# qiyu3816/DiffSG

Hardware: AMD Instinct MI355X
Metric: ddpm_reverse_sample_steps_per_sec_msr80c (higher is better)
Workload: dtype f32(2xf16-split MFMA, f32 accumulate); 1 GPU; MSR-80c CFG reverse sampling, batch 65536 x D=C=80 per GPU, UNet1D(proj 128, dims (64,32,16,8), n_blocks 2), omega=1, device Philox noise; rows sharded, no collective; batch_per_gpu=65536, solution_dim=80, parallelism=rows x1

## Files before the change

### diffsg_amd/csrc/dsg_panel.hpp

```cpp
#pragma once
#include "dsg_wide.hpp"

namespace dsg {

constexpr int kPW = 8;
constexpr int kPanelU4 = 2048;
constexpr int kPrivU4 = 128;
constexpr int kPrivSlots = 5;
constexpr int kPrivDist = 4;
constexpr int kPanelLdsU4 = 2 * kPanelU4 + kPW * kPrivSlots * kPrivU4 + kWideVec / 4;
constexpr int panel_pw(int steps) { return 2 * steps; }
constexpr int panel_u4(int steps) { return 512 * steps; }
constexpr int panel_lds_u4(int steps) { return 2 * panel_u4(steps) + panel_pw(steps) * kPrivSlots * kPrivU4 + kWideVec / 4; }

#ifndef DSG_STAMP_DBG
#define DSG_STAMP_DBG 0
#endif
#ifndef DSG_STAMP_DOWN0
#define DSG_STAMP_DOWN0 0
#endif
#ifdef DSG_CYCLE_STAMPS
constexpr int kPanelStampU4 = kPW * 128 / 2;
#define DSG_PSTAMP(tag)                                                                                               \
    do {                                                                                                              \
        if (STAMPED && blockIdx.x == 0 && stamp_k < 128) {                                                           \
            const unsigned long long t_ = __builtin_readcyclecounter();                                               \
            if (lane == 0 && !(DSG_STAMP_DBG & 1)) stamp_lds[wave * 128 + stamp_k] = (t_ << 16) | (unsigned long long)(tag); \
            if (DSG_STAMP_DBG & 1) asm volatile("" :: "s"(t_));                                                       \
            ++stamp_k;                                                                                                \
        }                                                                                                             \
    } while (0)
#else
constexpr int kPanelStampU4 = 0;
#define DSG_PSTAMP(tag) do {} while (0)
#endif

__device__ __forceinline__ void glds_quad_s(unsigned voff, const void* sbase, unsigned lds_dst) {
    unsigned keep;
    asm volatile("s_mov_b32 %0, m0\n\ts_mov_b32 m0, %3\n\ts_nop 0\n\t"
                 "global_load_lds_dwordx4 %1, %2\n\t"
                 "global_load_lds_dwordx4 %1, %2 offset:1024\n\t"
                 "global_load_lds_dwordx4 %1, %2 offset:2048\n\t"
                 "global_load_lds_dwordx4 %1, %2 offset:3072\n\t"
                 "s_mov_b32 m0, %0"
                 : "=&s"(keep) : "v"(voff), "s"(sbase), "s"(lds_dst) : "memory");
}
__device__ __forceinline__ void glds_pair_s(unsigned voff, const void* sbase, unsigned lds_dst) {
    unsigned keep;
    asm volatile("s_mov_b32 %0, m0\n\ts_mov_b32 m0, %3\n\ts_nop 0\n\t"
                 "global_load_lds_dwordx4 %1, %2\n\t"
                 "global_load_lds_dwordx4 %1, %2 offset:1024\n\t"
                 "s_mov_b32 m0, %0"
                 : "=&s"(keep) : "v"(voff), "s"(sbase), "s"(lds_dst) : "memory");
}
__device__ __forceinline__ void glds_stats_s(unsigned voff4, const void* s0, const void* s1, unsigned lds_dst) {
    unsigned keep;
    const void* s1m = reinterpret_cast<const char*>(s1) - 256;
    asm volatile("s_mov_b32 %0, m0\n\ts_mov_b32 m0, %4\n\ts_nop 0\n\t"
                 "global_load_lds_dword %1, %2\n\t"
                 "global_load_lds_dword %1, %3 offset:256\n\t"
                 "s_mov_b32 m0, %0"
                 : "=&s"(keep) : "v"(voff4), "s"(s0), "s"(s1m), "s"(lds_dst) : "memory");
}

struct TilePtrs {
    const char *x0, *x1, *cp;
    const char *st0, *st1;
    bool cond;
};
template <bool SCLIN, int PW = kPW>
__device__ __forceinline__ TilePtrs tile_ptrs(const BlockArgs& a, int g, int wave) {
    const int traw = g * PW + wave;
    const int tile = traw < a.ntiles ? traw : a.ntiles - 1;
    const int ptile = tile >= a.tiles_per_pass ? tile - a.tiles_per_pass : tile;
    const int t0 = seg_tile(a.in0, tile), t1 = seg_tile(a.in1, tile);
    TilePtrs t;
    t.x0 = reinterpret_cast<const char*>(a.in0.data + (size_t)t0 * 16 * 256);
    t.st0 = reinterpret_cast<const char*>(a.in0.stats + (size_t)t0 * 64);
    t.x1 = SCLIN ? reinterpret_cast<const char*>(a.in1.data + (size_t)t1 * 16 * 256) : t.x0;
    t.st1 = SCLIN ? reinterpret_cast<const char*>(a.in1.stats + (size_t)t1 * 64) : t.st0;
    t.cp = reinterpret_cast<const char*>(a.cond_pre + (size_t)ptile * 16 * 256);
    t.cond = tile >= a.uncond_tiles;
    return t;
}

struct PanelCtx {
    unsigned lane16, lane4;
    unsigned w_lds;
    unsigned w_rd;
    unsigned p_lds;
    const uint4* wrd;
    const uint4* prd;
    int q;
    int islot, cslot;
};

__device__ __forceinline__ void priv_issue(PanelCtx& c, const char* src) {
    glds_pair_s(c.lane16, src, c.p_lds + (unsigned)c.islot * 2048u);
    c.islot = c.islot == kPrivSlots - 1 ? 0 : c.islot + 1;
}
__device__ __forceinline__ void priv_issue_stats(PanelCtx& c, const char* st0, const char* st1) {
    glds_stats_s(c.lane4, st0, st1, c.p_lds + (unsigned)c.islot * 2048u);
    c.islot = c.islot == kPrivSlots - 1 ? 0 : c.islot + 1;
}
__device__ __forceinline__ const uint4* priv_consume(PanelCtx& c) {
    asm volatile("s_waitcnt vmcnt(6)" ::: "memory");
    const uint4* rd = c.prd + c.cslot * kPrivU4;
    c.cslot = c.cslot == kPrivSlots - 1 ? 0 : c.cslot + 1;
    return rd;
}

template <int NT>
__device__ __forceinline__ void panel_wfrag(HFrag<NT>& w, const uint4* panel , int steps_per_tile, int s) {
#pragma unroll
    for (int nt = 0; nt < NT; ++nt) { w.hi[nt] = panel[(nt * steps_per_tile + s) * 128]; w.lo[nt] = panel[(nt * steps_per_tile + s) * 128 + 64]; }
// ... 150 lines not shown
    if (HASN) {
        constexpr int L0 = 4 * NJ;
        asm volatile("" : "+v"(hq[L0 + 3]), "+v"(lq[L0 + 3]));
        const f32x4 hv = {hq[L0], hq[L0 + 1], hq[L0 + 2], hq[L0 + 3]}, lv = {lq[L0], lq[L0 + 1], lq[L0 + 2], lq[L0 + 3]};
        bcarry.hi = __builtin_bit_cast(h8, hv); bcarry.lo = __builtin_bit_cast(h8, lv);
    }
}

#ifndef DSG_PANEL_TRAIL_PRIO
#define DSG_PANEL_TRAIL_PRIO 1
#endif

template <int STEPS, bool STAMPED>
struct PanelWg {
    static constexpr int N = 128, NT = 4, NG = 16;
    static constexpr int PW = panel_pw(STEPS), PU4 = panel_u4(STEPS), NTHR = 64 * PW;
    static constexpr float kL2 = -1.44269504088896341f;
    int lane, h, j, wave;
    float *g1v, *b1v, *g2v, *b2v, *g3v, *b3v, *tbv, *c2v, *c3v, *gLv, *bLv, *biasLv;
    PanelCtx c;
    int since_w;
#ifdef DSG_CYCLE_STAMPS
    unsigned long long* stamp_lds;
    int stamp_k;
    unsigned long long clk_t0, clk_r0;
#endif
    __device__ __forceinline__ void stamp(int tag) { DSG_PSTAMP(tag); }

    __device__ __forceinline__ void init(uint4* lds) {
        lane = threadIdx.x & 63; h = lane >> 5; j = lane & 31;
        wave = __builtin_amdgcn_readfirstlane(threadIdx.x >> 6);
#ifdef DSG_CYCLE_STAMPS
        stamp_lds = reinterpret_cast<unsigned long long*>(lds + panel_lds_u4(STEPS));
        stamp_k = 0;
        clk_t0 = __builtin_readcyclecounter(); clk_r0 = __builtin_amdgcn_s_memrealtime();
#endif
        if (STEPS == 4 && wave >= 4) __builtin_amdgcn_s_setprio(DSG_PANEL_TRAIL_PRIO);
        float* const vec = reinterpret_cast<float*>(lds + 2 * PU4 + PW * kPrivSlots * kPrivU4);
        float* const v2 = vec + 2 * kLnLdsW1;
        g1v = vec; b1v = vec + kLnLdsW1;
        g2v = v2; b2v = v2 + 128; g3v = v2 + 256; b3v = v2 + 384; tbv = v2 + 512; c2v = v2 + 640; c3v = v2 + 768;
        gLv = v2 + 896; bLv = v2 + 1024; biasLv = v2 + 1152;
        const unsigned lds0 = (unsigned)(unsigned long long)(const __attribute__((address_space(3))) void*)lds;
        c.lane16 = (unsigned)lane * 16u; c.lane4 = (unsigned)lane * 4u;
        c.w_lds = lds0 + (unsigned)wave * 4096u;
        c.w_rd = lds0 + (unsigned)lane * 16u;
        c.p_lds = lds0 + 2u * PU4 * 16u + (unsigned)wave * (kPrivSlots * 2048u);
        c.wrd = lds + lane;
        c.prd = lds + 2 * PU4 + wave * (kPrivSlots * kPrivU4) + lane;
        c.q = 0; c.islot = 0; c.cslot = 0;
        since_w = 0;
    }

    template <typename More>
    __device__ __forceinline__ void stage_vectors(const BlockArgs& a, More&& more) {
        const int n1 = ln1_extent(a);
        for (int i = threadIdx.x; i < n1; i += NTHR) { g1v[i] = a.gamma1[i] * kL2; b1v[i] = a.beta1[i] * kL2; }
        if (threadIdx.x < 128) {
            const int i = threadIdx.x;
            g2v[i] = a.gamma2[i] * kL2; b2v[i] = a.beta2[i] * kL2; g3v[i] = a.gamma3[i] * kL2; b3v[i] = a.beta3[i] * kL2;
            c2v[i] = a.c2[i]; c3v[i] = a.c3[i];
            tbv[i] = a.tbias[(size_t)(a.step_ptr ? *a.step_ptr : 0) * a.tb_stride + i];
            more(i);
        }
        __syncthreads();
    }

    __device__ __forceinline__ void prologue(const char* st0, const char* st1, const char* x0, const uint4* panel0) {
        priv_issue_stats(c, st0, st1);
        priv_issue(c, x0);
        priv_issue(c, x0 + 2048);
        priv_issue(c, x0 + 4096);
        glds_quad_s(c.lane16, panel0, c.w_lds);
    }

    __device__ __forceinline__ int panel_begin(const uint4* next) {
        if (since_w >= 8) asm volatile("s_waitcnt vmcnt(8) lgkmcnt(0)" ::: "memory");
        else if (STEPS < 4 && since_w >= 4) asm volatile("s_waitcnt vmcnt(4) lgkmcnt(0)" ::: "memory");
        else if (since_w >= 2) asm volatile("s_waitcnt vmcnt(2) lgkmcnt(0)" ::: "memory");
        else asm volatile("s_waitcnt vmcnt(0) lgkmcnt(0)" ::: "memory");
        __builtin_amdgcn_s_barrier();
        const int rd = c.q & 1;
        glds_quad_s(c.lane16, next, c.w_lds + (unsigned)((c.q + 1) & 1) * (PU4 * 16u));
        since_w = 0;
        ++c.q;
        return rd;
    }

    __device__ __forceinline__ BOp step0_mem(const uint4* rd, const float* gv, const float* bv, float cc, float dd) {
        const float4 xa = __builtin_bit_cast(float4, rd[0]), xb = __builtin_bit_cast(float4, rd[64]);
        const float x[8] = {xa.x, xa.y, xa.z, xa.w, xb.x, xb.y, xb.z, xb.w};
        return panel_prep<true, true>(x, gv, bv, 0, cc, dd, h);
    }
    __device__ __forceinline__ BOp step0_reg(const f32x16 (&in)[NT], const float* gv, const float* bv, float cc, float dd) {
        const float x[8] = {in[0][0], in[0][1], in[0][2], in[0][3], in[0][4], in[0][5], in[0][6], in[0][7]};
        return panel_prep<true, true>(x, gv, bv, 0, cc, dd, h);
    }
    static __device__ __forceinline__ const uint4* no_consume(int) { return nullptr; }
    static __device__ __forceinline__ const uint4* none_n() { return nullptr; }

    template <int P1, typename Consume, typename Refill>
    __device__ __forceinline__ void stage1(f32x16 (&acc1)[NT], BOp b0, float cc, float dd, Consume&& consume_s1, Refill&& refill) {
#pragma unroll
        for (int p = 0; p < P1; ++p) {
            const int bi = panel_begin(refill(p));
            stamp(0x14);
            BOp bc;
            const NextPrep nx{&acc1, STEPS * (p + 1), g1v, b1v, cc, dd, nullptr, nullptr};
            auto cs = [&](int jj) { return consume_s1(STEPS * p + 1 + jj); };
            auto cn = [&]() { return consume_s1(STEPS * p + STEPS); };
            if (p + 1 < P1) {
                if (p == 0) panel_pipe_s<true, PIPE_LN, PIPE_LN, STEPS>(acc1, c.wrd + bi * PU4, b0, bc, acc1, STEPS * p, g1v, b1v, cc, dd, h, cs, nx, cn);
                else panel_pipe_s<false, PIPE_LN, PIPE_LN, STEPS>(acc1, c.wrd + bi * PU4, b0, bc, acc1, STEPS * p, g1v, b1v, cc, dd, h, cs, nx, cn);
                b0 = bc;
            } else {
                if (p == 0) panel_pipe_s<true, PIPE_LN, PIPE_NONE, STEPS>(acc1, c.wrd + bi * PU4, b0, bc, acc1, STEPS * p, g1v, b1v, cc, dd, h, cs, nx, none_n);
                else panel_pipe_s<false, PIPE_LN, PIPE_NONE, STEPS>(acc1, c.wrd + bi * PU4, b0, bc, acc1, STEPS * p, g1v, b1v, cc, dd, h, cs, nx, none_n);
            }
// ... 42 lines not shown
    template <typename Ahead>
    __device__ __forceinline__ void priv_add8(f32x16 (&acc)[NT], Ahead&& ahead) {
#pragma unroll
        for (int i = 0; i < 8; ++i) {
            const uint4* rd = priv_consume(c);
            const float4 v0 = __builtin_bit_cast(float4, rd[0]), v1 = __builtin_bit_cast(float4, rd[64]);
            ahead(i);
            acc_add_f4<NT>(acc, 2 * i, v0);
            acc_add_f4<NT>(acc, 2 * i + 1, v1);
        }
    }

    __device__ __forceinline__ void stats_store(const f32x16 (&acc)[NT], const BlockArgs& a, int tile, bool store, float& xmean, float& xm2) {
        acc_stats<N, NT>(acc, h, xmean, xm2);
        if (store) {
            if (h == 0) reinterpret_cast<float2*>(a.out_stats)[(size_t)tile * 32 + j] = make_float2(xmean, xm2);
            acc_store<NG, NT>(acc, a.out + (size_t)tile * NG * 256 + lane * 4);
        }
    }

    __device__ __forceinline__ void finish() {
        asm volatile("s_waitcnt vmcnt(0)" ::: "memory");
#ifdef DSG_CYCLE_STAMPS
        if (STAMPED && blockIdx.x == 0) {
            asm volatile("s_waitcnt lgkmcnt(0)" ::: "memory");
            for (int k = lane; k < 128; k += 64) dsg_stamp_buf[wave * 128 + k] = k < stamp_k ? stamp_lds[wave * 128 + k] : 0ull;
            if (threadIdx.x == 0) {
                dsg_stamp_buf[kPW * 128 + 0] = clk_t0; dsg_stamp_buf[kPW * 128 + 1] = clk_r0;
                dsg_stamp_buf[kPW * 128 + 2] = __builtin_readcyclecounter(); dsg_stamp_buf[kPW * 128 + 3] = __builtin_amdgcn_s_memrealtime();
                dsg_stamp_n = kPW * 128 + 4;
            }
        }
#endif
    }
};

template <bool SCLIN, int EPI, int NTO, int STEPS = 4>
__global__ __launch_bounds__(64 * panel_pw(STEPS), 2) void k_panel128_h(const BlockLinArgsH A, const int ngroups) {
    constexpr int NT = 4;
    constexpr int PW = panel_pw(STEPS), PU4 = panel_u4(STEPS);
    constexpr int KS1 = SCLIN ? 16 : 8, P1 = KS1 / STEPS, P2 = 8 / STEPS, NE = SCLIN ? 16 : 8;
    constexpr int NTOP = NTO <= 1 ? 1 : (NTO == 2 ? 2 : 4), ESTEPS = 4 * STEPS / NTOP;
    constexpr int EPANELS = EPI == 0 ? 0 : (ESTEPS >= 8 ? 1 : 8 / ESTEPS);
    constexpr int PA = P1, PB = PA + P2, PD = PB + P2, PE = PD + (SCLIN ? P1 : 0), NP = PE + EPANELS;
    __shared__ uint4 lds[panel_lds_u4(STEPS) + (STEPS == 4 ? kPanelStampU4 : 0)];
    PanelWg<STEPS, ((DSG_STAMP_DOWN0 ? !SCLIN : SCLIN) && EPI == 0 && STEPS == 4)> w;
    w.init(lds);
    PanelCtx& c = w.c;
    int& since_w = w.since_w;
    const BlockArgsH& ah = A.b;
    const BlockArgs& a = ah.b;
    const int lane = w.lane, h = w.h, j = w.j, wave = w.wave;
    const int stride = gridDim.x;
    w.stage_vectors(a, [&](int i) {
        if (EPI == 2) { w.gLv[i] = A.l.l.gamma[i] * w.kL2; w.bLv[i] = A.l.l.beta[i] * w.kL2; }
        if (EPI != 0) w.biasLv[i] = i < NTO * 32 ? A.l.l.bias[i] : 0.f;
    });
    const float inv1 = ah.kc[0], inv2 = ah.kc[1], inv3 = ah.kc[2];
    float invL = 0.f;
    if (EPI != 0) invL = A.l.kc[EPI == 2 ? 1 : 0];

    const int wnt = wave / (STEPS / 2), wsub = wave % (STEPS / 2);
    const uint4* const w1p = ah.W1h + ((size_t)wnt * KS1) * 128 + wsub * 256;
    const uint4* const w2p = ah.W2h + ((size_t)wnt * 8) * 128 + wsub * 256;
    const uint4* const w3p = ah.W3h + ((size_t)wnt * 8) * 128 + wsub * 256;
    const uint4* const wsp = SCLIN ? ah.Wsch + ((size_t)wnt * KS1) * 128 + wsub * 256 : w1p;
    const uint4* wlp = w1p;
    if (EPI != 0) {
        if (NTOP == 4) wlp = A.l.Wh + ((size_t)(wnt < NTO ? wnt : 0) * 8) * 128 + wsub * 256;
        else if (NTOP == 2) wlp = A.l.Wh + ((size_t)(wave / STEPS) * 8) * 128 + (wave % STEPS) * 256;
        else wlp = A.l.Wh + (wave & 3) * 256;
    }
    auto panel_src = [&](int p) -> const uint4* {
        if (p < PA) return w1p + (size_t)p * (128 * STEPS);
        if (p < PB) return w2p + (size_t)(p - PA) * (128 * STEPS);
        if (p < PD) return w3p + (size_t)(p - PB) * (128 * STEPS);
        if (p < PE) return wsp + (size_t)(p - PD) * (128 * STEPS);
        return wlp + (ESTEPS < 8 ? (size_t)(p - PE) * (128 * ESTEPS) : 0);
    };
    {
        const TilePtrs cur = tile_ptrs<SCLIN, PW>(a, blockIdx.x < ngroups ? blockIdx.x : 0, wave);
        w.prologue(cur.st0, cur.st1, cur.x0, panel_src(0));
    }
    auto xin = [&](const TilePtrs& t, int S) -> const char* { return SCLIN && S >= 8 ? t.x1 + (size_t)(S - 8) * 2048 : t.x0 + (size_t)S * 2048; };

    constexpr bool XT = SCLIN && EPI == 0;
    BOp bcar;
    float cc_car = 0.f, dd_car = 0.f;
    for (int g = blockIdx.x; g < ngroups; g += stride) {
        const int tile_raw = g * PW + wave;
        const bool live = tile_raw < a.ntiles;
        const int tile = live ? tile_raw : a.ntiles - 1;
        const int ptile = tile >= a.tiles_per_pass ? tile - a.tiles_per_pass : tile;
        const TilePtrs cur = tile_ptrs<SCLIN, PW>(a, g, wave);
        const bool my_cond = cur.cond;
        const TilePtrs nxt = tile_ptrs<SCLIN, PW>(a, g + stride < ngroups ? g + stride : g, wave);
        w.stamp(0x01);
        auto issue_tail = [&](int T) {
            if (T < NE) priv_issue(c, xin(cur, T));
            else if (T == NE) priv_issue_stats(c, nxt.st0, nxt.st1);
            else priv_issue(c, nxt.x0 + (size_t)(T - NE - 1) * 2048);
            since_w += 2;
        };
        auto consume_s1 = [&](int S) -> const uint4* {
            const uint4* rd = priv_consume(c);
            if (S + 4 < KS1) { priv_issue(c, xin(cur, S + 4)); since_w += 2; }
            else if (my_cond) { priv_issue(c, cur.cp + (size_t)(S + 4 - KS1) * 2048); since_w += 2; }
            else issue_tail(S + 4 - KS1);
            return rd;
        };
        auto consume_sc = [&](int S) -> const uint4* {
            const uint4* rd = priv_consume(c);
            issue_tail(S + 4);
            return rd;
        };

        auto ln1_stats = [&](const TilePtrs& t, float& cc, float& dd) {
            const uint4* rd = priv_consume(c);
            const float2* sp = reinterpret_cast<const float2*>(rd - lane);
            const float2 s0 = sp[j];
            float mean = s0.x, m2 = s0.y;
            if (SCLIN) {
                const float2 s1 = sp[32 + j];
                const float dd_ = s1.x - mean;
                m2 = m2 + s1.y + dd_ * dd_ * a.chan_w;
                mean = mean + dd_ * a.chan_f;
            }
            priv_issue(c, t.x0 + 3 * 2048); since_w += 2;
            const float rstd = rsqrtf(m2 * a.inv_nin + kLnEps);
            if (SCLIN) range_check(a.range_flag, mean, m2);
            cc = rstd; dd = -mean * rstd;
        };

        f32x16 acc1[NT];
        {
            float cc, dd;
// ... 106 lines not shown
                if (S == 0) mfma_step_h0<NTO>(acc, wf, bhi, blo); else mfma_step_h<NTO>(acc, wf, bhi, blo);
            }
        }
        acc_unscale_add_lds<NTO>(acc, invL, w.biasLv, h);
        if (!live) continue;
        if (EPI == 1) {
            const int NGo = (la.out_width + 7) / 8;
            float m, sq;
            lin_out_stats<NTO>(acc, h, la.out_width, la.inv_out_w, m, sq);
            if (h == 0) reinterpret_cast<float2*>(la.out_stats)[(size_t)tile * 32 + j] = make_float2(m, sq);
#pragma unroll
            for (int G = 0; G < NTO * 4; ++G)
                if (G < NGo) st4(la.out + ((size_t)tile * NGo + G) * 256 + lane * 4, acc_f4<NTO>(acc, G));
        } else {
            const int pass = tile >= la.tiles_per_pass ? 1 : 0, row = ptile * 32 + j;
            if (row < la.nrows) {
                float* o = la.out_rm + ((size_t)pass * la.nrows + row) * la.out_width;
                if ((la.out_width & 3) == 0) {
#pragma unroll
                    for (int G = 0; G < NTO * 4; ++G) {
                        const int f = 8 * G + 4 * h;
                        if (f < la.out_width) st4(o + f, acc_f4<NTO>(acc, G));
                    }
                } else {
#pragma unroll
                    for (int G = 0; G < NTO * 4; ++G)
#pragma unroll
                        for (int qq = 0; qq < 4; ++qq) {
                            const int f = 8 * G + 4 * h + qq;
                            if (f < la.out_width) o[f] = acc[G >> 2][4 * (G & 3) + qq];
                        }
                }
            }
        }
    }
    w.finish();
}

template <int STEPS = 4>
__global__ __launch_bounds__(64 * panel_pw(STEPS), 2) void k_panel128_duo_h(const BlockArgsH ah, const int ngroups) {
    constexpr int NT = 4;
    constexpr int PW = panel_pw(STEPS);
    constexpr int P = 8 / STEPS;
    constexpr int PA = P, PB = 2 * P, PD = 3 * P, NP = 4 * P;
    __shared__ uint4 lds[panel_lds_u4(STEPS) + (STEPS == 4 ? kPanelStampU4 : 0)];
    PanelWg<STEPS, (DSG_STAMP_DOWN0 && STEPS == 4)> w;
    w.init(lds);
    PanelCtx& c = w.c;
    int& since_w = w.since_w;
    const BlockArgs& a = ah.b;
    const int lane = w.lane, h = w.h, j = w.j, wave = w.wave;
    const int stride = gridDim.x;
    const int tpp = a.tiles_per_pass;
    w.stage_vectors(a, [](int) {});
    const float inv1 = ah.kc[0], inv2 = ah.kc[1], inv3 = ah.kc[2];

    const int wnt = wave / (STEPS / 2), wsub = wave % (STEPS / 2);
    const uint4* const w1p = ah.W1h + ((size_t)wnt * 8) * 128 + wsub * 256;
    const uint4* const w2p = ah.W2h + ((size_t)wnt * 8) * 128 + wsub * 256;
    const uint4* const w3p = ah.W3h + ((size_t)wnt * 8) * 128 + wsub * 256;
    auto panel_src = [&](int p) -> const uint4* {
        if (p < PA) return w1p + (size_t)p * (128 * STEPS);
        if (p < PB) return w2p + (size_t)(p - PA) * (128 * STEPS);
        if (p < PD) return w3p + (size_t)(p - PB) * (128 * STEPS);
        return w3p + (size_t)(p - PD) * (128 * STEPS);
    };
    struct RowPtrs { const char *x0, *st0, *cp; };
    auto row_ptrs = [&](int g) -> RowPtrs {
        const int raw = g * PW + wave, pt = raw < tpp ? raw : tpp - 1;
        return RowPtrs{reinterpret_cast<const char*>(a.in0.data + (size_t)pt * 16 * 256), reinterpret_cast<const char*>(a.in0.stats + (size_t)pt * 64),
                       reinterpret_cast<const char*>(a.cond_pre + (size_t)pt * 16 * 256)};
    };
    {
        const RowPtrs cur = row_ptrs(blockIdx.x < ngroups ? blockIdx.x : 0);
        w.prologue(cur.st0, cur.st0, cur.x0, panel_src(0));
    }

    for (int g = blockIdx.x; g < ngroups; g += stride) {
        const int row_raw = g * PW + wave;
        const bool live = row_raw < tpp;
        const int ptile = live ? row_raw : tpp - 1;
        const RowPtrs cur = row_ptrs(g);
        const RowPtrs nxt = row_ptrs(g + stride < ngroups ? g + stride : g);
        w.stamp(0x01);
        auto issue_at = [&](int T) {
            if (T < 8) priv_issue(c, cur.x0 + (size_t)T * 2048);
            else if (T < 16) priv_issue(c, cur.cp + (size_t)(T - 8) * 2048);
            else if (T < 24) priv_issue(c, cur.x0 + (size_t)(T - 16) * 2048);
            else if (T == 24) priv_issue_stats(c, nxt.st0, nxt.st0);
            else priv_issue(c, nxt.x0 + (size_t)(T - 25) * 2048);
            since_w += 2;
        };
        auto consume_s1 = [&](int S) -> const uint4* {
            const uint4* rd = priv_consume(c);
            if (S + 4 < 8) { priv_issue(c, cur.x0 + (size_t)(S + 4) * 2048); since_w += 2; }
            else issue_at(S + 4 - 8);
            return rd;
        };

        f32x16 acc1[NT];
        {
            float cc, dd;
            {
                const uint4* rd = priv_consume(c);
                const float2 s0 = reinterpret_cast<const float2*>(rd - lane)[j];
                priv_issue(c, cur.x0 + 3 * 2048); since_w += 2;
                const float rstd = rsqrtf(s0.y * a.inv_nin + kLnEps);
                cc = rstd; dd = -s0.x * rstd;
            }
            w.stamp(0x10);
            BOp b0 = w.step0_mem(consume_s1(0), w.g1v, w.b1v, cc, dd);
            asm volatile("" : "+v"(b0.hi), "+v"(b0.lo));
            w.stamp(0x11);
            w.template stage1<P>(acc1, b0, cc, dd, consume_s1, [&](int p) { return panel_src(p + 1); });
        }
        acc_unscale_add_lds<NT>(acc1, inv1, w.tbv, h);
        w.stamp(0x13);

        f32x16 acc2[NT];
        {
            float cc, dd;
            BOp b0 = w.template reg_head<0x20>(acc1, w.g2v, w.b2v, cc, dd);
            w.template reg_panels<P - 1, 0x20>(acc2, acc1, w.g2v, w.b2v, cc, dd, b0, [&](int p) { return panel_src(PA + p + 1); });
            w.template reg_last<0x20>(acc2, acc1, w.g2v, w.b2v, cc, dd, b0, panel_src(PA + P));
            acc_unscale_add_lds<NT>(acc2, inv2, w.c2v, h);
        }
        w.stamp(0x23);

        f32x16 (&acc3)[NT] = acc1;
// ... 91 lines not shown
```

### diffsg_amd/csrc/dsg_res64.hpp

```cpp
#pragma once
#include "dsg_panel.hpp"

namespace dsg {

constexpr int kR64Waves = 8;
typedef unsigned u32x4 __attribute__((ext_vector_type(4)));
typedef __attribute__((address_space(3))) const u32x4 lds_cu4;

template <bool SCLIN, int NTO = 0> struct R64Layout {
    static constexpr int KS1 = SCLIN ? 8 : 4;
    static constexpr int W1 = 0, W2 = W1 + 2 * KS1 * 128, W3 = W2 + 2 * 4 * 128, WSC = W3 + 2 * 4 * 128, WL = WSC + (SCLIN ? 2 * KS1 * 128 : 0),
                         VEC = WL + NTO * 4 * 128;
    static constexpr int G1 = 0, B1 = 16 * KS1, G2 = 2 * 16 * KS1, B2 = G2 + 64, G3 = B2 + 64, B3 = G3 + 64, TB = B3 + 64, C2 = TB + 64, C3 = C2 + 64,
                         BL = C3 + 64, NV = BL + 32 * NTO;
    static constexpr int TOTAL_U4 = VEC + (NV + 3) / 4;
};

template <bool LNACT>
__device__ __forceinline__ void r64_prep(const float (&x)[8], const float* gv, const float* bv, int S, float c, float d, int h, h8& hi, h8& lo) {
    const BOp o = panel_prep<LNACT>(x, gv, bv, S, c, d, h);
    hi = o.hi; lo = o.lo;
}

struct R64Planes { u32x4 h0, l0, h1, l1; };
__device__ __forceinline__ R64Planes r64_planes(lds_cu4* w, int tile_stride) { return R64Planes{w[0], w[64], w[tile_stride], w[tile_stride + 64]}; }
struct R64Vec { f32x4 g0, b0, g1, b1; };
__device__ __forceinline__ R64Vec r64_vec(const float* gv, const float* bv, int S, int h) {
    lds_cf4* const gl = (lds_cf4*)(gv + 4 * h);
    lds_cf4* const bl = (lds_cf4*)(bv + 4 * h);
    return R64Vec{gl[4 * S], bl[4 * S], gl[4 * S + 2], bl[4 * S + 2]};
}
template <bool FIRST>
__device__ __forceinline__ void r64_mma_p(f32x16 (&acc)[2], const R64Planes& p, const h8 bhi, const h8 blo) {
    if (FIRST) {
        const f32x16 z = {0.f, 0.f, 0.f, 0.f, 0.f, 0.f, 0.f, 0.f, 0.f, 0.f, 0.f, 0.f, 0.f, 0.f, 0.f, 0.f};
        acc[0] = __builtin_amdgcn_mfma_f32_32x32x16_f16(__builtin_bit_cast(h8, p.h0), bhi, z, 0, 0, 0);
        acc[1] = __builtin_amdgcn_mfma_f32_32x32x16_f16(__builtin_bit_cast(h8, p.h1), bhi, z, 0, 0, 0);
    } else {
        DSG_MFMA_H(acc[0], __builtin_bit_cast(h8, p.h0), bhi);
        DSG_MFMA_H(acc[1], __builtin_bit_cast(h8, p.h1), bhi);
    }
    DSG_MFMA_H(acc[0], __builtin_bit_cast(h8, p.h0), blo);
    DSG_MFMA_H(acc[1], __builtin_bit_cast(h8, p.h1), blo);
    DSG_MFMA_H(acc[0], __builtin_bit_cast(h8, p.l0), bhi);
    DSG_MFMA_H(acc[1], __builtin_bit_cast(h8, p.l1), bhi);
}
template <bool LNACT>
__device__ __forceinline__ void r64_prep_v(const float (&x)[8], const R64Vec& vv, float c, float d, h8& hi, h8& lo) {
    float v[8];
    if (LNACT) {
        constexpr float kk = -1.44269504088896341f / kActScale;
        const float g[8] = {vv.g0[0], vv.g0[1], vv.g0[2], vv.g0[3], vv.g1[0], vv.g1[1], vv.g1[2], vv.g1[3]};
        const float b[8] = {vv.b0[0], vv.b0[1], vv.b0[2], vv.b0[3], vv.b1[0], vv.b1[1], vv.b1[2], vv.b1[3]};
#pragma unroll
        for (int q = 0; q < 8; ++q) {
            const float u = fmaf(fmaf(x[q], c, d), g[q], b[q]);
            v[q] = u * __builtin_amdgcn_rcpf(fmaf(__builtin_amdgcn_exp2f(u), kk, kk));
        }
// ... 38 lines not shown
                __builtin_amdgcn_sched_group_barrier(0x008, 1, 0);
                __builtin_amdgcn_sched_group_barrier(0x002, LNACT ? 11 : 4, 0);
            }
        }
        __builtin_amdgcn_sched_barrier(0);
        pc = pn; bh = nh; bl = nl;
    }
}

template <int NQ>
__device__ __forceinline__ void r64_unscale_add(f32x16 (&acc)[2], float inv, const float* vec, int h) {
    lds_cf4* const v = (lds_cf4*)(vec + 4 * h);
#pragma unroll
    for (int nt = 0; nt < 2; ++nt)
#pragma unroll
        for (int q = 0; q < 4; ++q) {
            const f32x4 b = v[8 * nt + 2 * q];
            acc[nt][4 * q + 0] = fmaf(acc[nt][4 * q + 0], inv, b[0]); acc[nt][4 * q + 1] = fmaf(acc[nt][4 * q + 1], inv, b[1]);
            acc[nt][4 * q + 2] = fmaf(acc[nt][4 * q + 2], inv, b[2]); acc[nt][4 * q + 3] = fmaf(acc[nt][4 * q + 3], inv, b[3]);
        }
}

struct R64Tile {
    const float *x0, *x1, *cp;
    const float2 *st0, *st1;
    bool cond;
};
template <bool SCLIN>
__device__ __forceinline__ R64Tile r64_tile(const BlockArgs& a, int g, int wave, int lane, int j) {
    const int traw = g * kR64Waves + wave;
    const int tile = traw < a.ntiles ? traw : a.ntiles - 1;
    const int ptile = tile >= a.tiles_per_pass ? tile - a.tiles_per_pass : tile;
    const int t0 = seg_tile(a.in0, tile), t1 = seg_tile(a.in1, tile);
    R64Tile t;
    t.x0 = a.in0.data + (size_t)t0 * 8 * 256 + lane * 4;
    t.st0 = reinterpret_cast<const float2*>(a.in0.stats) + (size_t)t0 * 32 + j;
    t.x1 = SCLIN ? a.in1.data + (size_t)t1 * 8 * 256 + lane * 4 : t.x0;
    t.st1 = SCLIN ? reinterpret_cast<const float2*>(a.in1.stats) + (size_t)t1 * 32 + j : t.st0;
    t.cp = a.cond_pre + (size_t)ptile * 8 * 256 + lane * 4;
    t.cond = tile >= a.uncond_tiles;
    return t;
}

template <bool SCLIN, int NTO>
struct R64Staged {
    static constexpr int KS1 = R64Layout<SCLIN, NTO>::KS1, N1 = 2 * KS1 * 128 / 512, N2 = 2 * 4 * 128 / 512, NL = (NTO * 4 * 128 + 511) / 512;
    uint4 r1[N1], r2[N2], r3[N2], rs[SCLIN ? N1 : 1], rl[NTO > 0 ? NL : 1];
    float g1, b1, bl, v6[6], tb;
};
template <bool SCLIN, int NTO>
__device__ __forceinline__ void r64_staged_load(R64Staged<SCLIN, NTO>& s, const BlockArgsH& ah, const LinArgsH* lin , int tid) {
    using S = R64Staged<SCLIN, NTO>;
    const BlockArgs& a = ah.b;
    s.g1 = 0.f; s.b1 = 0.f; s.bl = 0.f; s.tb = 0.f;
#pragma unroll
    for (int q = 0; q < 6; ++q) s.v6[q] = 0.f;
#pragma unroll
    for (int k = 0; k < S::N1; ++k) s.r1[k] = ah.W1h[tid + 512 * k];
#pragma unroll
    for (int k = 0; k < S::N2; ++k) { s.r2[k] = ah.W2h[tid + 512 * k]; s.r3[k] = ah.W3h[tid + 512 * k]; }
    if constexpr (SCLIN) {
#pragma unroll
        for (int k = 0; k < S::N1; ++k) s.rs[k] = ah.Wsch[tid + 512 * k];
    }
    if constexpr (NTO > 0) {
#pragma unroll
        for (int k = 0; k < S::NL; ++k) {
            s.rl[k] = make_uint4(0u, 0u, 0u, 0u);
            if (512 * (k + 1) <= NTO * 4 * 128 || tid + 512 * k < NTO * 4 * 128) s.rl[k] = lin->Wh[tid + 512 * k];
        }
        if (tid < 32 * NTO) s.bl = lin->l.bias[tid];
    }
    if (tid < 16 * S::KS1) { s.g1 = a.gamma1[tid]; s.b1 = a.beta1[tid]; }
    if (tid < 64) {
        s.v6[0] = a.gamma2[tid]; s.v6[1] = a.beta2[tid]; s.v6[2] = a.gamma3[tid]; s.v6[3] = a.beta3[tid]; s.v6[4] = a.c2[tid]; s.v6[5] = a.c3[tid];
        s.tb = a.tbias[(size_t)(a.step_ptr ? *a.step_ptr : 0) * a.tb_stride + tid];
    }
}
template <bool SCLIN, int NTO>
__device__ __forceinline__ void r64_staged_write(const R64Staged<SCLIN, NTO>& s, uint4* lb, int tid) {
    using S = R64Staged<SCLIN, NTO>;
    using L = R64Layout<SCLIN, NTO>;
    constexpr float kL2 = -1.44269504088896341f;
    float* const vec = reinterpret_cast<float*>(lb + L::VEC);
#pragma unroll
    for (int k = 0; k < S::N1; ++k) lb[L::W1 + tid + 512 * k] = s.r1[k];
#pragma unroll
    for (int k = 0; k < S::N2; ++k) { lb[L::W2 + tid + 512 * k] = s.r2[k]; lb[L::W3 + tid + 512 * k] = s.r3[k]; }
    if constexpr (SCLIN) {
#pragma unroll
        for (int k = 0; k < S::N1; ++k) lb[L::WSC + tid + 512 * k] = s.rs[k];
    }
    if constexpr (NTO > 0) {
#pragma unroll
        for (int k = 0; k < S::NL; ++k)
            if (512 * (k + 1) <= NTO * 4 * 128 || tid + 512 * k < NTO * 4 * 128) lb[L::WL + tid + 512 * k] = s.rl[k];
        if (tid < 32 * NTO) vec[L::BL + tid] = s.bl;
    }
    if (tid < 16 * S::KS1) { vec[L::G1 + tid] = s.g1 * kL2; vec[L::B1 + tid] = s.b1 * kL2; }
    if (tid < 64) {
        vec[L::G2 + tid] = s.v6[0] * kL2; vec[L::B2 + tid] = s.v6[1] * kL2; vec[L::G3 + tid] = s.v6[2] * kL2; vec[L::B3 + tid] = s.v6[3] * kL2;
        vec[L::C2 + tid] = s.v6[4]; vec[L::C3 + tid] = s.v6[5];
        vec[L::TB + tid] = s.tb;
    }
}

template <int XG>
__device__ __forceinline__ auto r64_x_regs(const float4 (&xc)[XG]) {
    return [&xc](int S, float (&x)[8]) {
        x[0] = xc[2 * S].x; x[1] = xc[2 * S].y; x[2] = xc[2 * S].z; x[3] = xc[2 * S].w;
        x[4] = xc[2 * S + 1].x; x[5] = xc[2 * S + 1].y; x[6] = xc[2 * S + 1].z; x[7] = xc[2 * S + 1].w;
    };
}
__device__ __forceinline__ auto r64_x_acc(const f32x16 (&in)[2]) {
    return [&in](int S, float (&x)[8]) {
        const int t = S >> 1, r0 = 8 * (S & 1);
#pragma unroll
        for (int q = 0; q < 8; ++q) x[q] = in[t][r0 + q];
    };
}

template <typename L, int XG>
__device__ __forceinline__ void r64_stages(f32x16 (&acc3)[2], const float4 (&xc)[XG], float mean1, float rstd1, uint4* lb, float inv1, float inv2,
                                           bool cond, const float* cp, int lane, int h) {
    constexpr int N = 64, NT = 2, NG = 8, KS1 = L::KS1;
    lds_cu4* const w1 = (lds_cu4*)(lb + L::W1) + lane;
    lds_cu4* const w2 = (lds_cu4*)(lb + L::W2) + lane;
    lds_cu4* const w3 = (lds_cu4*)(lb + L::W3) + lane;
    const float* const vec = reinterpret_cast<const float*>(lb + L::VEC);
    float4 cpv[NG];
    if (cond) {
#pragma unroll
        for (int G = 0; G < NG; ++G) cpv[G] = ld4(cp + (size_t)G * 256);
    }
    f32x16 (&acc1)[NT] = acc3;
    r64_stage<true, true, KS1>(acc1, w1, KS1 * 128, vec + L::G1, vec + L::B1, rstd1, -mean1 * rstd1, h, r64_x_regs<XG>(xc), [](int) {});
    r64_unscale_add<8>(acc1, inv1, vec + L::TB, h);
    f32x16 acc2[NT];
    {
        float mean, m2;
        acc_stats<N, NT>(acc1, h, mean, m2);
        const float rstd = rsqrtf(m2 * (1.0f / N) + kLnEps);
        r64_stage<true, true, 4>(acc2, w2, 4 * 128, vec + L::G2, vec + L::B2, rstd, -mean * rstd, h, r64_x_acc(acc1), [](int) {});
        r64_unscale_add<8>(acc2, inv2, vec + L::C2, h);
    }
    if (cond) {
#pragma unroll
        for (int G = 0; G < NG; ++G) acc_add_f4<NT>(acc2, G, cpv[G]);
    }
    {
        float mean, m2;
        acc_stats<N, NT>(acc2, h, mean, m2);
        const float rstd = rsqrtf(m2 * (1.0f / N) + kLnEps);
        r64_stage<true, true, 4>(acc3, w3, 4 * 128, vec + L::G3, vec + L::B3, rstd, -mean * rstd, h, r64_x_acc(acc2), [](int) {});
    }
}

__device__ __forceinline__ int r64_opaque_lane(int lane) {
    asm volatile("" : "+v"(lane));
    return lane;
}
__device__ __forceinline__ void r64_stats_store(const f32x16 (&acc)[2], const BlockArgs& a, int tile, bool store, int lane_o, int h, float& xmean,
                                                float& xm2) {
    acc_stats<64, 2>(acc, h, xmean, xm2);
    if (store) {
        if (lane_o < 32) reinterpret_cast<float2*>(a.out_stats)[(size_t)tile * 32 + lane_o] = make_float2(xmean, xm2);
        acc_store<8, 2>(acc, a.out + (size_t)tile * 8 * 256 + lane_o * 4);
    }
}

template <typename L, typename Next>
__device__ __forceinline__ void r64_plain_block(f32x16 (&acc3)[2], const float4 (&xc)[8], float2 sc, uint4* lb, const BlockArgs& a, const float (&inv)[3], bool cond,
                                                const float* cp, int tile, bool store, int lane, int lane_o, int h, float& xmean, float& xm2,
                                                Next&& next_input) {
    r64_stages<L, 8>(acc3, xc, sc.x, rsqrtf(sc.y * a.inv_nin + kLnEps), lb, inv[0], inv[1], cond, cp, lane, h);
    r64_unscale_add<8>(acc3, inv[2], reinterpret_cast<const float*>(lb + L::VEC) + L::C3, h);
    next_input();
#pragma unroll
    for (int G = 0; G < 8; ++G) acc_add_f4<2>(acc3, G, xc[G]);
    r64_stats_store(acc3, a, tile, store, lane_o, h, xmean, xm2);
}

template <bool SCLIN, int NTO>
__global__ __launch_bounds__(512, 2) void k_res64_lds(const BlockLinArgsH A, const int ngroups) {
    using L = R64Layout<SCLIN, NTO>;
    const BlockArgsH& ah = A.b;
    constexpr int NT = 2, KS1 = L::KS1, XG = SCLIN ? 16 : 8;
    __shared__ uint4 lds[L::TOTAL_U4];
    float* const vec = reinterpret_cast<float*>(lds + L::VEC);
    const BlockArgs& a = ah.b;
    const int lane = threadIdx.x & 63, h = lane >> 5, j = lane & 31;
    const int wave = __builtin_amdgcn_readfirstlane(threadIdx.x >> 6);
    {
        R64Staged<SCLIN, NTO> s;
        r64_staged_load(s, ah, &A.l, threadIdx.x);
        r64_staged_write(s, lds, threadIdx.x);
    }
    const float inv[3] = {ah.kc[0], ah.kc[1], ah.kc[2]};
    float invL = 0.f;
    if (NTO > 0) invL = A.l.kc[0];
    __syncthreads();
    lds_cu4* const wl = (lds_cu4*)(lds + L::WL) + lane;
    lds_cu4* const wsc = (lds_cu4*)(lds + L::WSC) + lane;
    auto xsrc = [&](const R64Tile& t, int G) -> const float* { return SCLIN && G >= 8 ? t.x1 + (size_t)(G - 8) * 256 : t.x0 + (size_t)G * 256; };

    float4 xc[XG];
    float2 s0c, s1c;
    {
        const R64Tile t = r64_tile<SCLIN>(a, blockIdx.x < ngroups ? blockIdx.x : 0, wave, lane, j);
#pragma unroll
        for (int G = 0; G < XG; ++G) xc[G] = ld4(xsrc(t, G));
        s0c = *t.st0; s1c = *t.st1;
    }

    for (int g = blockIdx.x; g < ngroups; g += gridDim.x) {
        asm volatile("" ::: "memory");
        const int tile_raw = g * kR64Waves + wave;
        const bool live = tile_raw < a.ntiles;
        const int tile = live ? tile_raw : a.ntiles - 1;
        const R64Tile cur = r64_tile<SCLIN>(a, g, wave, lane, j);
        const R64Tile nxt = r64_tile<SCLIN>(a, g + gridDim.x < ngroups ? g + gridDim.x : g, wave, lane, j);
        const int lane_o = r64_opaque_lane(lane);
        const bool store = live && (NTO == 0 || A.store_block_out);
        f32x16 acc3[NT];
        float xmean, xm2;
        float4 xn[XG];
        float2 s0n, s1n;
        if constexpr (!SCLIN) {
            r64_plain_block<L>(acc3, xc, s0c, lds, a, inv, cur.cond, cur.cp, tile, store, lane, lane_o, h, xmean, xm2, [&]() {
                s0n = *nxt.st0; s1n = s0n;
#pragma unroll
                for (int G = 0; G < XG; ++G) xn[G] = ld4(xsrc(nxt, G));
            });
        } else {
            const float dm = s1c.x - s0c.x;
            const float m2 = s0c.y + s1c.y + dm * dm * a.chan_w;
            const float mean1 = s0c.x + dm * a.chan_f;
            const float rstd1 = rsqrtf(m2 * a.inv_nin + kLnEps);
            range_check(a.range_flag, mean1, m2);
            r64_stages<L, XG>(acc3, xc, mean1, rstd1, lds, inv[0], inv[1], cur.cond, cur.cp, lane, h);
            s0n = *nxt.st0; s1n = *nxt.st1;
            r64_stage<false, false, KS1>(acc3, wsc, KS1 * 128, nullptr, nullptr, 0.f, 0.f, h, r64_x_regs<XG>(xc),
                                         [&](int S) { xn[2 * S] = ld4(xsrc(nxt, 2 * S)); xn[2 * S + 1] = ld4(xsrc(nxt, 2 * S + 1)); });
            r64_unscale_add<8>(acc3, inv[2], vec + L::C3, h);
            r64_stats_store(acc3, a, tile, store, lane_o, h, xmean, xm2);
        }
        if constexpr (NTO > 0) {
            range_check(a.range_flag, xmean, xm2);
            const LinArgs& la = A.l.l;
            f32x16 accL[NTO];
#pragma unroll
            for (int S = 0; S < 4; ++S) {
                const int t = S >> 1, r0 = 8 * (S & 1);
                const float x[8] = {acc3[t][r0], acc3[t][r0 + 1], acc3[t][r0 + 2], acc3[t][r0 + 3], acc3[t][r0 + 4], acc3[t][r0 + 5], acc3[t][r0 + 6], acc3[t][r0 + 7]};
                h8 bhi, blo;
                r64_prep<false>(x, nullptr, nullptr, 0, 0.f, 0.f, h, bhi, blo);
                HFrag<NTO> w;
#pragma unroll
                for (int nt = 0; nt < NTO; ++nt) {
                    const u32x4 hh = wl[(nt * 4 + S) * 128], ll = wl[(nt * 4 + S) * 128 + 64];
                    w.hi[nt] = __builtin_bit_cast(uint4, hh); w.lo[nt] = __builtin_bit_cast(uint4, ll);
                }
                if (S == 0) mfma_step_h0<NTO>(accL, w, bhi, blo); else mfma_step_h<NTO>(accL, w, bhi, blo);
            }
            {
                lds_cf4* const v = (lds_cf4*)(vec + L::BL + 4 * h);
#pragma unroll
                for (int nt = 0; nt < NTO; ++nt)
#pragma unroll
                    for (int q = 0; q < 4; ++q) {
                        const f32x4 b = v[8 * nt + 2 * q];
                        accL[nt][4 * q + 0] = fmaf(accL[nt][4 * q + 0], invL, b[0]); accL[nt][4 * q + 1] = fmaf(accL[nt][4 * q + 1], invL, b[1]);
                        accL[nt][4 * q + 2] = fmaf(accL[nt][4 * q + 2], invL, b[2]); accL[nt][4 * q + 3] = fmaf(accL[nt][4 * q + 3], invL, b[3]);
                    }
            }
            if (live) {
                const int NGo = (la.out_width + 7) / 8;
                float sm = 0.f;
#pragma unroll
                for (int G = 0; G < NTO * 4; ++G)
#pragma unroll
                    for (int qq = 0; qq < 4; ++qq)
                        if (8 * G + 4 * h + qq < la.out_width) sm += accL[G >> 2][4 * (G & 3) + qq];
                const float m = xhalf_sum(sm) * la.inv_out_w;
                float sq = 0.f;
#pragma unroll
                for (int G = 0; G < NTO * 4; ++G)
#pragma unroll
                    for (int qq = 0; qq < 4; ++qq)
                        if (8 * G + 4 * h + qq < la.out_width) { const float dv = accL[G >> 2][4 * (G & 3) + qq] - m; sq = fmaf(dv, dv, sq); }
                sq = xhalf_sum(sq);
                if (lane_o < 32) reinterpret_cast<float2*>(la.out_stats)[(size_t)tile * 32 + lane_o] = make_float2(m, sq);
#pragma unroll
                for (int G = 0; G < NTO * 4; ++G)
                    if (G < NGo) st4(la.out + ((size_t)tile * NGo + G) * 256 + lane_o * 4, acc_f4<NTO>(accL, G));
            }
        }
#pragma unroll
        for (int G = 0; G < XG; ++G) xc[G] = xn[G];
        s0c = s0n; s1c = s1n;
    }
}

__global__ __launch_bounds__(512, 2) void k_res64_dual(const BlockArgsH A0, const BlockArgsH A1, const int ngroups) {
    using L = R64Layout<false, 0>;
    constexpr int NT = 2, NG = 8;
    __shared__ uint4 lds[2 * L::TOTAL_U4];
    const int lane = threadIdx.x & 63, h = lane >> 5, j = lane & 31;
    const int wave = __builtin_amdgcn_readfirstlane(threadIdx.x >> 6);
    {
        R64Staged<false, 0> s0, s1;
        r64_staged_load(s0, A0, nullptr, threadIdx.x);
        r64_staged_load(s1, A1, nullptr, threadIdx.x);
        r64_staged_write(s0, lds, threadIdx.x);
        r64_staged_write(s1, lds + L::TOTAL_U4, threadIdx.x);
    }
    const float inv[2][3] = {{A0.kc[0], A0.kc[1], A0.kc[2]}, {A1.kc[0], A1.kc[1], A1.kc[2]}};
    __syncthreads();
    const BlockArgs& a0 = A0.b;
    float4 xc[NG];
    float2 sc;
    {
        const R64Tile t = r64_tile<false>(a0, blockIdx.x < ngroups ? blockIdx.x : 0, wave, lane, j);
#pragma unroll
        for (int G = 0; G < NG; ++G) xc[G] = ld4(t.x0 + (size_t)G * 256);
        sc = *t.st0;
    }
    for (int g = blockIdx.x; g < ngroups; g += gridDim.x) {
        asm volatile("" ::: "memory");
        const int tile_raw = g * kR64Waves + wave;
        const bool live = tile_raw < a0.ntiles;
        const int tile = live ? tile_raw : a0.ntiles - 1;
        const int ptile = tile >= a0.tiles_per_pass ? tile - a0.tiles_per_pass : tile;
        const bool cond = tile >= a0.uncond_tiles;
        const R64Tile nxt = r64_tile<false>(a0, g + gridDim.x < ngroups ? g + gridDim.x : g, wave, lane, j);
        const int lane_o = r64_opaque_lane(lane);
        float4 xn[NG];
        float2 sn = sc;
#pragma unroll
        for (int k = 0; k < 2; ++k) {
            const BlockArgs& a = k == 0 ? A0.b : A1.b;
            f32x16 acc3[NT];
            float xmean, xm2;
            r64_plain_block<L>(acc3, xc, sc, lds + k * L::TOTAL_U4, a, inv[k], cond, a.cond_pre + (size_t)ptile * NG * 256 + lane * 4, tile, live, lane,
                               lane_o, h, xmean, xm2, [&]() {
                                   if (k == 1) {
#pragma unroll
                                       for (int G = 0; G < NG; ++G) xn[G] = ld4(nxt.x0 + (size_t)G * 256);
                                       sn = *nxt.st0;
                                   }
                               });
            if (k == 0) {
#pragma unroll
                for (int G = 0; G < NG; ++G) xc[G] = acc_f4<NT>(acc3, G);
                sc = make_float2(xmean, xm2);
            }
        }
#pragma unroll
        for (int G = 0; G < NG; ++G) xc[G] = xn[G];
        sc = sn;
    }
}


}
```

Measured before the change: 1294 steps/s.

## Overlap kernel prologue vector staging with first tile loads

In the panel kernels, the per-layer LayerNorm and bias vector staging now runs after the first panel and tile prefetch has been issued. All vector loads are batched into registers ahead of the LDS writes, and the time-bias row is fetched with a direct global-to-LDS load. In the res64 kernels, the first input tile load is moved ahead of the staged LDS writes and barrier, and the branchy staged loads are made unconditional using modulo indexing. The aim is to hide global-load latency in each block's startup. The cost is more registers held live during startup, redundant duplicate loads and LDS writes, and more inline-asm fragility.

```diff
diff --git a/diffsg_amd/csrc/dsg_panel.hpp b/diffsg_amd/csrc/dsg_panel.hpp
--- a/diffsg_amd/csrc/dsg_panel.hpp
+++ b/diffsg_amd/csrc/dsg_panel.hpp
@@ -61,6 +61,13 @@
                  "global_load_lds_dword %1, %3 offset:256\n\t"
                  "s_mov_b32 m0, %0"
                  : "=&s"(keep) : "v"(voff4), "s"(s0), "s"(s1m), "s"(lds_dst) : "memory");
+}
+__device__ __forceinline__ void glds_row_s(unsigned voff4, const void* s0, unsigned lds_dst) {
+    unsigned keep;
+    asm volatile("s_mov_b32 %0, m0\n\ts_mov_b32 m0, %3\n\ts_nop 0\n\t"
+                 "global_load_lds_dword %1, %2\n\t"
+                 "s_mov_b32 m0, %0"
+                 : "=&s"(keep) : "v"(voff4), "s"(s0), "s"(lds_dst) : "memory");
 }
 
 struct TilePtrs {
@@ -317,18 +324,45 @@
         since_w = 0;
     }
 
-    template <typename More>
-    __device__ __forceinline__ void stage_vectors(const BlockArgs& a, More&& more) {
-        const int n1 = ln1_extent(a);
-        for (int i = threadIdx.x; i < n1; i += NTHR) { g1v[i] = a.gamma1[i] * kL2; b1v[i] = a.beta1[i] * kL2; }
-        if (threadIdx.x < 128) {
-            const int i = threadIdx.x;
-            g2v[i] = a.gamma2[i] * kL2; b2v[i] = a.beta2[i] * kL2; g3v[i] = a.gamma3[i] * kL2; b3v[i] = a.beta3[i] * kL2;
-            c2v[i] = a.c2[i]; c3v[i] = a.c3[i];
-            tbv[i] = a.tbias[(size_t)(a.step_ptr ? *a.step_ptr : 0) * a.tb_stride + i];
-            more(i);
-        }
-        __syncthreads();
+    static constexpr int NG1 = (kLnLdsW1 + NTHR - 1) / NTHR;
+    template <typename LoadMore, typename WriteMore>
+    __device__ __forceinline__ void stage_vectors(const BlockArgs& a, LoadMore&& load_more, WriteMore&& write_more) {
+        const int n1 = ln1_extent(a), i = (threadIdx.x + NTHR / 2) % NTHR;
+        const int vwave = (wave + PW / 2) % PW;
+        int zero = 0;
+        asm("" : "+v"(zero));
+        int step = (a.step_ptr ? a.step_ptr : reinterpret_cast<const int*>(a.tbias))[zero];
+        const unsigned step_bytes = a.step_ptr ? (unsigned)a.tb_stride * 4u : 0u;
+        float g1[NG1], b1[NG1], v6[6], m[3] = {0.f, 0.f, 0.f};
+#pragma unroll
+        for (int k = 0; k < NG1; ++k) {
+            g1[k] = 0.f; b1[k] = 0.f;
+            if (i + k * NTHR < n1) { g1[k] = a.gamma1[i + k * NTHR]; b1[k] = a.beta1[i + k * NTHR]; }
+        }
+#pragma unroll
+        for (int q = 0; q < 6; ++q) v6[q] = 0.f;
+        if (i < 128) {
+            v6[0] = a.gamma2[i]; v6[1] = a.beta2[i]; v6[2] = a.gamma3[i]; v6[3] = a.beta3[i]; v6[4] = a.c2[i]; v6[5] = a.c3[i];
+            load_more(i, m);
+        }
+        __builtin_amdgcn_sched_barrier(0);
+#pragma unroll
+        for (int k = 0; k < NG1; ++k)
+            if (i + k * NTHR < n1) { g1v[i + k * NTHR] = g1[k] * kL2; b1v[i + k * NTHR] = b1[k] * kL2; }
+        if (i < 128) {
+            g2v[i] = v6[0] * kL2; b2v[i] = v6[1] * kL2; g3v[i] = v6[2] * kL2; b3v[i] = v6[3] * kL2;
+            c2v[i] = v6[4]; c3v[i] = v6[5];
+            write_more(i, m);
+        }
+        stamp(0x03);
+        if (vwave < 2) {
+            const unsigned tb_lds = (unsigned)(unsigned long long)(const __attribute__((address_space(3))) void*)tbv;
+            asm volatile("" : "+v"(step));
+            glds_row_s(c.lane4 + (unsigned)step * step_bytes, a.tbias + vwave * 64, tb_lds + (unsigned)vwave * 256u);
+        }
+        asm volatile("s_waitcnt lgkmcnt(0)" ::: "memory");
+        __builtin_amdgcn_s_barrier();
+        stamp(0x04);
     }
 
     __device__ __forceinline__ void prologue(const char* st0, const char* st1, const char* x0, const uint4* panel0) {
@@ -477,13 +511,7 @@
     const BlockArgs& a = ah.b;
     const int lane = w.lane, h = w.h, j = w.j, wave = w.wave;
     const int stride = gridDim.x;
-    w.stage_vectors(a, [&](int i) {
-        if (EPI == 2) { w.gLv[i] = A.l.l.gamma[i] * w.kL2; w.bLv[i] = A.l.l.beta[i] * w.kL2; }
-        if (EPI != 0) w.biasLv[i] = i < NTO * 32 ? A.l.l.bias[i] : 0.f;
-    });
-    const float inv1 = ah.kc[0], inv2 = ah.kc[1], inv3 = ah.kc[2];
-    float invL = 0.f;
-    if (EPI != 0) invL = A.l.kc[EPI == 2 ? 1 : 0];
+    w.stamp(0x02);
 
     const int wnt = wave / (STEPS / 2), wsub = wave % (STEPS / 2);
     const uint4* const w1p = ah.W1h + ((size_t)wnt * KS1) * 128 + wsub * 256;
@@ -506,7 +534,20 @@
     {
         const TilePtrs cur = tile_ptrs<SCLIN, PW>(a, blockIdx.x < ngroups ? blockIdx.x : 0, wave);
         w.prologue(cur.st0, cur.st1, cur.x0, panel_src(0));
-    }
+        w.stamp(0x05);
+    }
+    w.stage_vectors(a,
+        [&](int i, float (&m)[3]) {
+            if (EPI == 2) { m[0] = A.l.l.gamma[i]; m[1] = A.l.l.beta[i]; }
+            if (EPI != 0) { if (i < NTO * 32) m[2] = A.l.l.bias[i]; }
+        },
+        [&](int i, const float (&m)[3]) {
+            if (EPI == 2) { w.gLv[i] = m[0] * w.kL2; w.bLv[i] = m[1] * w.kL2; }
+            if (EPI != 0) w.biasLv[i] = m[2];
+        });
+    const float inv1 = ah.kc[0], inv2 = ah.kc[1], inv3 = ah.kc[2];
+    float invL = 0.f;
+    if (EPI != 0) invL = A.l.kc[EPI == 2 ? 1 : 0];
     auto xin = [&](const TilePtrs& t, int S) -> const char* { return SCLIN && S >= 8 ? t.x1 + (size_t)(S - 8) * 2048 : t.x0 + (size_t)S * 2048; };
 
     constexpr bool XT = SCLIN && EPI == 0;
@@ -719,8 +760,7 @@
     const int lane = w.lane, h = w.h, j = w.j, wave = w.wave;
     const int stride = gridDim.x;
     const int tpp = a.tiles_per_pass;
-    w.stage_vectors(a, [](int) {});
-    const float inv1 = ah.kc[0], inv2 = ah.kc[1], inv3 = ah.kc[2];
+    w.stamp(0x02);
 
     const int wnt = wave / (STEPS / 2), wsub = wave % (STEPS / 2);
     const uint4* const w1p = ah.W1h + ((size_t)wnt * 8) * 128 + wsub * 256;
@@ -741,7 +781,10 @@
     {
         const RowPtrs cur = row_ptrs(blockIdx.x < ngroups ? blockIdx.x : 0);
         w.prologue(cur.st0, cur.st0, cur.x0, panel_src(0));
-    }
+        w.stamp(0x05);
+    }
+    w.stage_vectors(a, [](int, float (&)[3]) {}, [](int, const float (&)[3]) {});
+    const float inv1 = ah.kc[0], inv2 = ah.kc[1], inv3 = ah.kc[2];
 
     for (int g = blockIdx.x; g < ngroups; g += stride) {
         const int row_raw = g * PW + wave;
diff --git a/diffsg_amd/csrc/dsg_res64.hpp b/diffsg_amd/csrc/dsg_res64.hpp
--- a/diffsg_amd/csrc/dsg_res64.hpp
+++ b/diffsg_amd/csrc/dsg_res64.hpp
@@ -4,6 +4,9 @@
 namespace dsg {
 
 constexpr int kR64Waves = 8;
+#ifndef DSG_R64_FIRST_EARLY
+#define DSG_R64_FIRST_EARLY 1
+#endif
 typedef unsigned u32x4 __attribute__((ext_vector_type(4)));
 typedef __attribute__((address_space(3))) const u32x4 lds_cu4;
 
@@ -148,6 +151,7 @@
 __device__ __forceinline__ void r64_staged_load(R64Staged<SCLIN, NTO>& s, const BlockArgsH& ah, const LinArgsH* lin , int tid) {
     using S = R64Staged<SCLIN, NTO>;
     const BlockArgs& a = ah.b;
+    const int step = a.step_ptr ? *a.step_ptr : 0;
     s.g1 = 0.f; s.b1 = 0.f; s.bl = 0.f; s.tb = 0.f;
 #pragma unroll
     for (int q = 0; q < 6; ++q) s.v6[q] = 0.f;
@@ -165,13 +169,12 @@
             s.rl[k] = make_uint4(0u, 0u, 0u, 0u);
             if (512 * (k + 1) <= NTO * 4 * 128 || tid + 512 * k < NTO * 4 * 128) s.rl[k] = lin->Wh[tid + 512 * k];
         }
-        if (tid < 32 * NTO) s.bl = lin->l.bias[tid];
-    }
-    if (tid < 16 * S::KS1) { s.g1 = a.gamma1[tid]; s.b1 = a.beta1[tid]; }
-    if (tid < 64) {
-        s.v6[0] = a.gamma2[tid]; s.v6[1] = a.beta2[tid]; s.v6[2] = a.gamma3[tid]; s.v6[3] = a.beta3[tid]; s.v6[4] = a.c2[tid]; s.v6[5] = a.c3[tid];
-        s.tb = a.tbias[(size_t)(a.step_ptr ? *a.step_ptr : 0) * a.tb_stride + tid];
-    }
+        s.bl = lin->l.bias[tid % (32 * NTO)];
+    }
+    const int t1 = tid % (16 * S::KS1), t2 = tid % 64;
+    s.g1 = a.gamma1[t1]; s.b1 = a.beta1[t1];
+    s.v6[0] = a.gamma2[t2]; s.v6[1] = a.beta2[t2]; s.v6[2] = a.gamma3[t2]; s.v6[3] = a.beta3[t2]; s.v6[4] = a.c2[t2]; s.v6[5] = a.c3[t2];
+    s.tb = a.tbias[(size_t)step * a.tb_stride + t2];
 }
 template <bool SCLIN, int NTO>
 __device__ __forceinline__ void r64_staged_write(const R64Staged<SCLIN, NTO>& s, uint4* lb, int tid) {
@@ -191,14 +194,13 @@
 #pragma unroll
         for (int k = 0; k < S::NL; ++k)
             if (512 * (k + 1) <= NTO * 4 * 128 || tid + 512 * k < NTO * 4 * 128) lb[L::WL + tid + 512 * k] = s.rl[k];
-        if (tid < 32 * NTO) vec[L::BL + tid] = s.bl;
-    }
-    if (tid < 16 * S::KS1) { vec[L::G1 + tid] = s.g1 * kL2; vec[L::B1 + tid] = s.b1 * kL2; }
-    if (tid < 64) {
-        vec[L::G2 + tid] = s.v6[0] * kL2; vec[L::B2 + tid] = s.v6[1] * kL2; vec[L::G3 + tid] = s.v6[2] * kL2; vec[L::B3 + tid] = s.v6[3] * kL2;
-        vec[L::C2 + tid] = s.v6[4]; vec[L::C3 + tid] = s.v6[5];
-        vec[L::TB + tid] = s.tb;
-    }
+        vec[L::BL + tid % (32 * NTO)] = s.bl;
+    }
+    const int t1 = tid % (16 * S::KS1), t2 = tid % 64;
+    vec[L::G1 + t1] = s.g1 * kL2; vec[L::B1 + t1] = s.b1 * kL2;
+    vec[L::G2 + t2] = s.v6[0] * kL2; vec[L::B2 + t2] = s.v6[1] * kL2; vec[L::G3 + t2] = s.v6[2] * kL2; vec[L::B3 + t2] = s.v6[3] * kL2;
+    vec[L::C2 + t2] = s.v6[4]; vec[L::C3 + t2] = s.v6[5];
+    vec[L::TB + t2] = s.tb;
 }
 
 template <int XG>
@@ -287,27 +289,29 @@
     const BlockArgs& a = ah.b;
     const int lane = threadIdx.x & 63, h = lane >> 5, j = lane & 31;
     const int wave = __builtin_amdgcn_readfirstlane(threadIdx.x >> 6);
+    auto xsrc = [&](const R64Tile& t, int G) -> const float* { return SCLIN && G >= 8 ? t.x1 + (size_t)(G - 8) * 256 : t.x0 + (size_t)G * 256; };
+    constexpr bool FIRST_EARLY = DSG_R64_FIRST_EARLY == 2 || (DSG_R64_FIRST_EARLY == 1 && !SCLIN);
+    float4 xc[XG];
+    float2 s0c, s1c;
+    auto first_input = [&]() {
+        const R64Tile t = r64_tile<SCLIN>(a, blockIdx.x < ngroups ? blockIdx.x : 0, wave, lane, j);
+#pragma unroll
+        for (int G = 0; G < XG; ++G) xc[G] = ld4(xsrc(t, G));
+        s0c = *t.st0; s1c = *t.st1;
+    };
     {
         R64Staged<SCLIN, NTO> s;
         r64_staged_load(s, ah, &A.l, threadIdx.x);
+        if constexpr (FIRST_EARLY) first_input();
         r64_staged_write(s, lds, threadIdx.x);
     }
     const float inv[3] = {ah.kc[0], ah.kc[1], ah.kc[2]};
     float invL = 0.f;
     if (NTO > 0) invL = A.l.kc[0];
     __syncthreads();
+    if constexpr (!FIRST_EARLY) first_input();
     lds_cu4* const wl = (lds_cu4*)(lds + L::WL) + lane;
     lds_cu4* const wsc = (lds_cu4*)(lds + L::WSC) + lane;
-    auto xsrc = [&](const R64Tile& t, int G) -> const float* { return SCLIN && G >= 8 ? t.x1 + (size_t)(G - 8) * 256 : t.x0 + (size_t)G * 256; };
-
-    float4 xc[XG];
-    float2 s0c, s1c;
-    {
-        const R64Tile t = r64_tile<SCLIN>(a, blockIdx.x < ngroups ? blockIdx.x : 0, wave, lane, j);
-#pragma unroll
-        for (int G = 0; G < XG; ++G) xc[G] = ld4(xsrc(t, G));
-        s0c = *t.st0; s1c = *t.st1;
-    }
 
     for (int g = blockIdx.x; g < ngroups; g += gridDim.x) {
         asm volatile("" ::: "memory");
@@ -404,24 +408,26 @@
     __shared__ uint4 lds[2 * L::TOTAL_U4];
     const int lane = threadIdx.x & 63, h = lane >> 5, j = lane & 31;
     const int wave = __builtin_amdgcn_readfirstlane(threadIdx.x >> 6);
+    const BlockArgs& a0 = A0.b;
+    float4 xc[NG];
+    float2 sc;
+    auto first_input = [&]() {
+        const R64Tile t = r64_tile<false>(a0, blockIdx.x < ngroups ? blockIdx.x : 0, wave, lane, j);
+#pragma unroll
+        for (int G = 0; G < NG; ++G) xc[G] = ld4(t.x0 + (size_t)G * 256);
+        sc = *t.st0;
+    };
     {
         R64Staged<false, 0> s0, s1;
         r64_staged_load(s0, A0, nullptr, threadIdx.x);
         r64_staged_load(s1, A1, nullptr, threadIdx.x);
+        if constexpr (DSG_R64_FIRST_EARLY != 0) first_input();
         r64_staged_write(s0, lds, threadIdx.x);
         r64_staged_write(s1, lds + L::TOTAL_U4, threadIdx.x);
     }
     const float inv[2][3] = {{A0.kc[0], A0.kc[1], A0.kc[2]}, {A1.kc[0], A1.kc[1], A1.kc[2]}};
     __syncthreads();
-    const BlockArgs& a0 = A0.b;
-    float4 xc[NG];
-    float2 sc;
-    {
-        const R64Tile t = r64_tile<false>(a0, blockIdx.x < ngroups ? blockIdx.x : 0, wave, lane, j);
-#pragma unroll
-        for (int G = 0; G < NG; ++G) xc[G] = ld4(t.x0 + (size_t)G * 256);
-        sc = *t.st0;
-    }
+    if constexpr (DSG_R64_FIRST_EARLY == 0) first_input();
     for (int g = blockIdx.x; g < ngroups; g += gridDim.x) {
         asm volatile("" ::: "memory");
         const int tile_raw = g * kR64Waves + wave;
```

Result: faster. 1310 steps/s, median of 6 (+1.2%).
